# fircarpediem/LSS2_Multimodal_nu

Measured on AMD Instinct MI355X. Metric: BEV frames/sec (6-cam 352x128 -> 200x200x64), full hot path: CamEncode lift + splat + BevEncode, higher is better.
Workload: dtype bf16; 1 GPU; BASELINE configs[1]: model_BEV_TXT LSS hot path, batch=4/GPU, 6 cams 352x128, D=41, 200x200x64 BEV -> BevEncode -> 200x200x4, trunk (EfficientNet) not included: features are the input; batch_per_gpu=4, global_batch=4, parallelism=dp1 (sample-sharded, no collective), precision=bf16

## Files before the change

include/lss_hip.h:

```cpp
#ifndef LSS_HIP_H_
#define LSS_HIP_H_

#include <stddef.h>
#include <stdint.h>

#ifdef __cplusplus
extern "C" {
#endif

#define LSS_ABI_VERSION 1

#define LSS_E_NULL (-1)
#define LSS_E_SHAPE (-2)
#define LSS_E_LAYOUT (-3)
#define LSS_E_ALIGN (-4)
#define LSS_E_WORKSPACE (-5)
#define LSS_E_RCCL_BASE (-100)

#define LSS_BEV_NCHW_F32 0
#define LSS_BEV_NHWC_F32 1
#define LSS_BEV_NHWC_BF16 2

#define LSS_DT_F32 0
#define LSS_DT_BF16 1
// ... 72 lines not shown
                        int n_points, int C, void* workspace, size_t workspace_bytes, float* d_value,
                        float* d_offsets_logits, void* stream);
size_t lss_deform_attn_bwd_workspace_bytes(int B, int H, int W);

int lss_layernorm_fwd(const void* x, int x_dt, const float* gamma, const float* beta,
                      long long rows, int C, float eps, void* y, int y_dt, void* stream);

size_t lss_conv2d_packed_weight_bytes(int Cout, int Cin, int KH, int KW, int dt);
int lss_conv2d_pack_weights(const float* w_oihw, int Cout, int Cin, int KH, int KW,
                            int dt, void* w_packed, void* stream);
int lss_conv2d_fwd(const void* x, const void* x2, const void* w_packed,
                   const float* scale, const float* shift, const void* residual,
                   void* y, float* stats, int B, int H, int W, int Cx, int C2, int up,
                   int Cout, int KH, int KW, int stride, int pad, int relu, int dt,
                   void* stream);

int lss_conv2d_ring_ok(int B, int H, int W, int Cx, int C2, int up, int Cout, int head_n);
size_t lss_conv2d_ring_packed_weight_bytes(int Cout, int Cin);
int lss_conv2d_pack_weights_ring(const float* w_oihw, int Cout, int Cin, void* w_packed, void* stream);
int lss_conv2d_pack_weights_ring_dgrad(const float* w_oihw, int Cout, int Cin, void* w_packed, void* stream);
int lss_conv2d_ring_timeouts(void);

int lss_conv2d_ks_ok(int B, int H, int W, int Cin, int Cout);
size_t lss_conv2d_ks_packed_weight_bytes(int Cout, int Cin);
int lss_conv2d_pack_weights_ks(const float* w_oihw, int Cout, int Cin, void* w_packed, void* stream);
int lss_conv2d_pack_weights_ks_dgrad(const float* w_oihw, int Cout, int Cin, void* w_packed, void* stream);

int lss_conv2d_ks_s2_dual_ok(int B, int H, int W, int Cin, int Cout);
size_t lss_conv2d_ks_s2_dual_packed_weight_bytes(int Cout, int Cin);
int lss_conv2d_pack_weights_ks_s2_dual(const float* w1_oihw, const float* wd_oi, int Cout, int Cin, void* w_packed,
                                       void* stream);
int lss_conv2d_ks_s2_dual_fwd(const void* x, const void* w_packed, const float* scale, const float* shift, void* y,
                              void* y2, int B, int H, int W, int Cin, int Cout, int relu, void* stream);

int lss_conv2d_pack_weights_dgrad(const float* w_oihw, int Cout, int Cin, int KH, int KW, int dt,
                                  void* w_packed, void* stream);
size_t lss_conv2d_wgrad_workspace_bytes(int B, int H, int W, int Cin, int Cout);
int lss_conv2d_wgrad(const void* x, const void* dy, int B, int H, int W, int Cin, int Cout,
                     void* workspace, size_t workspace_bytes, float* dw_oihw, void* stream);
int lss_conv2d_wgrad_timeouts(void);
int lss_conv2d_s2_dgrad_taps(int K, int pad);
int lss_conv2d_pack_weights_s2_dgrad(const float* w_oihw, int Cout, int Cin, int K, int pad, void* w_packed, void* stream);
size_t lss_conv2d_wgrad4x4_workspace_bytes(int B, int H, int W, int Cin, int Cout);
int lss_conv2d_wgrad4x4(const void* xs, const void* dy, int B, int H, int W, int Cin, int Cout,
                        void* workspace, size_t workspace_bytes, float* dw16, void* stream);

int lss_upsample_cat_nhwc(const void* x, const void* x2, int B, int H, int W, int Cx, int C2, int up,
                          void* out, void* stream);
int lss_upsample_bwd_nhwc(const void* g, int B, int H, int W, int Cx, int Ct, int c_off, int up,
                          void* dx, void* stream);

size_t lss_bn_train_workspace_bytes(long long M, int C);
int lss_bn_train_fwd(const void* z, const void* residual, long long M, int C, const float* gamma,
                     const float* beta, float* running_mean, float* running_var, float momentum,
                     float eps, int relu, void* workspace, void* y, float* save_mean,
                     float* save_invstd, void* stream);
int lss_bn_train_bwd(const void* dy, const void* y, const void* z, long long M, int C,
                     const float* gamma, const float* save_mean, const float* save_invstd, int relu,
                     void* workspace, void* dz, void* dres, float* dgamma, float* dbeta, void* stream);

int lss_bn_partial_sums(const void* z, const void* dy, const void* y, const float* mean, const float* invstd,
                        long long M, int C, int relu, int mode, void* workspace, float* sums, void* stream);
int lss_bn_train_fwd_from_sums(const void* z, const void* residual, long long M, int C, const float* sums,
                               long long M_total, const float* gamma, const float* beta, float* running_mean,
                               float* running_var, float momentum, float eps, int relu, void* workspace,
                               void* y, float* save_mean, float* save_invstd, void* stream);
// ... 138 lines not shown
```

lss2_multimodal_nu_amd/_native.py:

```python
import ctypes
import os

import torch

_HERE = os.path.dirname(os.path.abspath(__file__))
LIB_PATH = os.environ.get("LSS_HIP_LIB") or os.path.join(_HERE, "csrc", "liblss_hip.so")

BEV_NCHW_F32, BEV_NHWC_F32, BEV_NHWC_BF16 = 0, 1, 2
DT_F32, DT_BF16 = 0, 1
ACT_NONE, ACT_RELU, ACT_GELU, OUT_F32, OUT_HEAD_MAJOR32, W_RING, W_KS = 0, 1, 2, 16, 32, 64, 128
VALUE_NHWC, VALUE_HEAD_MAJOR = 0, 1

_vp, _i, _sz = ctypes.c_void_p, ctypes.c_int, ctypes.c_size_t

SIGNATURES = {
    "lss_abi_version": (_i, []),
    "lss_error_string": (ctypes.c_char_p, [_i]),
    "lss_points_to_voxels": (_i, [_vp] * 7 + [_i] * 8 + [_vp, _vp, _vp, _vp]),
    "lss_geom_to_voxels": (_i, [_vp, _vp, _vp] + [_i] * 5 + [_vp, _vp, _vp]),
    "lss_bucket_points": (_i, [_vp, _vp, _i, _i, _i, _i, _vp, _vp, _vp, _vp, _vp]),
    "lss_depthnet_softmax_fwd": (_i, [_vp, _vp, _vp, _i, _i, _i, _i, _i, _vp, _vp, _i, _vp]),
    "lss_camencode_v2_fwd": (_i, [_vp, _i, _vp, _vp, _i, _vp, _vp, _vp] + [_i] * 7 + [_vp, _vp, _vp]),
    "lss_depth_fuse_softmax_fwd": (_i, [_vp] * 5 + [_i] * 6 + [_vp, _vp]),
    "lss_add_pos_fwd": (_i, [_vp, _vp, _i, _i, _i, _i, _vp, _vp]),
    "lss_deform_attn_fwd": (_i, [_vp, _i] + [_vp] * 4 + [_i] * 7 + [_vp, _vp]),
    "lss_deform_attn_pts_fwd": (_i, [_vp] * 3 + [ctypes.c_longlong] + [_i] * 6 + [_vp, _vp]),
    "lss_deform_attn_bwd": (_i, [_vp] * 3 + [ctypes.c_longlong, _vp] + [_i] * 6 + [_vp, _sz, _vp, _vp, _vp]),
    "lss_deform_attn_bwd_workspace_bytes": (_sz, [_i] * 3),
    "lss_layernorm_fwd": (_i, [_vp, _i, _vp, _vp, ctypes.c_longlong, _i, ctypes.c_float, _vp, _i, _vp]),
    "lss_depthnet_voxels_fwd": (_i, [_vp] * 10 + [_i] * 10 + [_vp] * 5),
    "lss_linear_res_ln_fwd": (_i, [_vp] * 4 + [ctypes.c_longlong, _i, _vp, _vp, _vp, ctypes.c_float, _vp, _vp]),
    "lss_ffn_fused_fwd": (_i, [_vp] * 5 + [ctypes.c_longlong, _i, _i, _vp, _vp, _vp, ctypes.c_float, _vp, _vp]),
    "lss_depthnet_voxels_hostcal_fwd": (_i, [_vp] * 7 + [_i] * 10 + [_vp] * 5),
    "lss_lift_splat_forward_hostcal": (_i, [_vp] * 7 + [_i] * 10 + [_vp] * 8 + [_i, _vp]),
    "lss_lift_splat_fwd": (_i, [_vp] * 3 + [_i] * 9 + [_vp, _i, _vp]),
    "lss_lift_splat_bwd": (_i, [_vp, _i, _vp, _vp, _vp] + [_i] * 9 + [_vp, _vp]),
    "lss_segmented_sum": (_i, [_vp, _vp, _i, _i, _vp, _vp]),
    "lss_conv2d_packed_weight_bytes": (_sz, [_i] * 5),
    "lss_conv2d_pack_weights": (_i, [_vp, _i, _i, _i, _i, _i, _vp, _vp]),
    "lss_conv2d_fwd": (_i, [_vp] * 8 + [_i] * 13 + [_vp]),
    "lss_conv2d_ring_ok": (_i, [_i] * 8),
    "lss_conv2d_ring_packed_weight_bytes": (_sz, [_i, _i]),
    "lss_conv2d_pack_weights_ring": (_i, [_vp, _i, _i, _vp, _vp]),
    "lss_conv2d_pack_weights_ring_dgrad": (_i, [_vp, _i, _i, _vp, _vp]),
    "lss_conv2d_ks_ok": (_i, [_i] * 5),
    "lss_conv2d_ks_packed_weight_bytes": (_sz, [_i, _i]),
    "lss_conv2d_pack_weights_ks": (_i, [_vp, _i, _i, _vp, _vp]),
    "lss_conv2d_pack_weights_ks_dgrad": (_i, [_vp, _i, _i, _vp, _vp]),
    "lss_conv2d_ks_s2_dual_ok": (_i, [_i] * 5),
    "lss_conv2d_ks_s2_dual_packed_weight_bytes": (_sz, [_i, _i]),
    "lss_conv2d_pack_weights_ks_s2_dual": (_i, [_vp, _vp, _i, _i, _vp, _vp]),
    "lss_conv2d_ks_s2_dual_fwd": (_i, [_vp] * 6 + [_i] * 6 + [_vp]),
    "lss_gather_pack": (_i, [_vp, _i, _vp]),
    "lss_conv_bn_act_train_pack": (_i, [_vp] + [_i] * 8 + [_vp, _vp]),
    "lss_clip_adam_partials": (ctypes.c_longlong, [_vp, _i]),
    "lss_clip_adam_step": (_i, [_vp, _i, _vp, _vp, ctypes.c_longlong] + [ctypes.c_float] * 6 + [_vp]),
    "lss_conv2d_wgrad_timeouts": (_i, []),
    "lss_conv2d_ring_timeouts": (_i, []),
    "lss_conv2d_pack_weights_dgrad": (_i, [_vp, _i, _i, _i, _i, _i, _vp, _vp]),
    "lss_conv2d_wgrad_workspace_bytes": (_sz, [_i] * 5),
    "lss_conv2d_wgrad": (_i, [_vp, _vp, _i, _i, _i, _i, _i, _vp, _sz, _vp, _vp]),
    "lss_conv2d_wgrad4x4_workspace_bytes": (_sz, [_i] * 5),
    "lss_conv2d_s2_dgrad_taps": (_i, [_i, _i]),
    "lss_conv2d_pack_weights_s2_dgrad": (_i, [_vp, _i, _i, _i, _i, _vp, _vp]),
    "lss_conv2d_wgrad4x4": (_i, [_vp, _vp, _i, _i, _i, _i, _i, _vp, _sz, _vp, _vp]),
    "lss_upsample_cat_nhwc": (_i, [_vp, _vp, _i, _i, _i, _i, _i, _i, _vp, _vp]),
    "lss_upsample_bwd_nhwc": (_i, [_vp, _i, _i, _i, _i, _i, _i, _i, _vp, _vp]),
    "lss_bn_train_workspace_bytes": (_sz, [ctypes.c_longlong, _i]),
    "lss_bn_train_fwd": (_i, [_vp, _vp, ctypes.c_longlong, _i, _vp, _vp, _vp, _vp, ctypes.c_float, ctypes.c_float, _i,
                              _vp, _vp, _vp, _vp, _vp]),
    "lss_bn_train_bwd": (_i, [_vp, _vp, _vp, ctypes.c_longlong, _i, _vp, _vp, _vp, _i, _vp, _vp, _vp, _vp, _vp, _vp]),
    "lss_bn_partial_sums": (_i, [_vp] * 5 + [ctypes.c_longlong, _i, _i, _i, _vp, _vp, _vp]),
    "lss_bn_train_fwd_from_sums": (_i, [_vp, _vp, ctypes.c_longlong, _i, _vp, ctypes.c_longlong, _vp, _vp, _vp, _vp,
                                        ctypes.c_float, ctypes.c_float, _i, _vp, _vp, _vp, _vp, _vp]),
    "lss_bn_train_bwd_from_sums": (_i, [_vp, _vp, _vp, ctypes.c_longlong, _i, _vp, ctypes.c_longlong, _vp, _vp, _vp, _i,
                                        _vp, _vp, _vp, _vp, _vp, _vp]),
    "lss_conv_bn_act_train_fwd": (_i, [_vp] * 14 + [_i] * 7 + [ctypes.c_float, ctypes.c_float, _i, _vp]),
    "lss_conv_bn_act_train_bwd": (_i, [_vp] * 11 + [_sz] + [_vp] * 9 + [_i] * 8 + [_vp]),
    "lss_weighted_ce_fwd": (_i, [_vp, _vp, _vp, _i, _i, ctypes.c_longlong, _vp, _vp, _vp, _vp]),
    "lss_weighted_ce_bwd": (_i, [_vp, _vp, _vp, _i, _i, ctypes.c_longlong, _vp, _vp, _vp, _vp]),
    "lss_conv2d_s2d_packed_weight_bytes": (_sz, [_i] * 4),
    "lss_conv2d_pack_weights_s2d": (_i, [_vp, _i, _i, _i, _i, _vp, _vp]),
    "lss_conv2d_s2_fwd": (_i, [_vp] * 7 + [_i] * 8 + [_vp]),
    "lss_conv2d_head_fwd": (_i, [_vp] * 8 + [_i] * 9 + [_vp]),
    "lss_conv2d_s2_dual_fwd": (_i, [_vp] * 6 + [_i] * 9 + [_vp]),
# ... 101 lines not shown
```

lss2_multimodal_nu_amd/csrc/conv_ks.hip:

```cpp
#include <stdlib.h>

#include "lss_common.h"

namespace {

constexpr int KS_ROWS = 7;
constexpr int KS_POSB = 64;
constexpr int KS_LDS_MAX = 160 * 1024;

__device__ __attribute__((aligned(128))) unsigned char lss_ks_zero_page[128];

__device__ __forceinline__ void ks_glds16(const void* gsrc, void* lds_wave_base) {
  __builtin_amdgcn_global_load_lds((const __attribute__((address_space(1))) void*)gsrc,
                                   (__attribute__((address_space(3))) void*)lds_wave_base, 16, 0, 0);
}

struct KsArgs {
  const unsigned short* x;
  const unsigned char* w;
  const float* scale;
  const float* shift;
  const unsigned short* residual;
  unsigned short* y;
  int B, H, W, Cin, Cout, relu, wt;
// ... 517 lines not shown
  const int patch = (Cin / 32) * p.nposp * KS_POSB;
  if (patch > 112 * 1024) return p;
  const int red = 2 * p.nkw * (p.PB / 16) * KS2_CT * 1024;
  p.lds = patch > red ? patch : red;
  if (p.lds > KS_LDS_MAX) return p;
  const long long grid = (long long)B * p.npb * p.ncb;
  if (grid < 64 || grid > 512) return p;
  if ((long long)B * H * W * Cin >= (1LL << 30) || (long long)B * HWo * Cout >= (1LL << 30)) return p;
  p.grid = (int)grid;
  p.ok = 1;
  return p;
}

template <int NKW>
int ks_s2_launch(const KsS2Plan& p, const KsS2Args& a, hipStream_t st) {
  static bool attr_set[64] = {};
  int dev = -1;
  if (hipGetDevice(&dev) != hipSuccess || dev < 0 || dev >= 64) dev = -1;
  if (dev < 0 || !attr_set[dev]) {
    hipError_t e = hipFuncSetAttribute(reinterpret_cast<const void*>(conv_ks_s2_dual_kernel<NKW>),
                                       hipFuncAttributeMaxDynamicSharedMemorySize, KS_LDS_MAX);
    if (e != hipSuccess) return (int)e;
    if (dev >= 0) attr_set[dev] = true;
  }
  hipLaunchKernelGGL((conv_ks_s2_dual_kernel<NKW>), dim3(p.grid), dim3(256), p.lds, st, a);
  return lss_launch_status();
}

unsigned long long* ks_stamps_from_env() {
  const char* e = getenv("LSS_KS_STAMPS");
  return e ? reinterpret_cast<unsigned long long*>(strtoull(e, nullptr, 16)) : nullptr;
}

}

extern "C" int lss_conv2d_ks_ok(int B, int H, int W, int Cin, int Cout) {
  if (const char* e = getenv("LSS_CONV_KS"))
    if (atoi(e) == 0) return 0;
  return ks_plan(B, H, W, Cin, Cout).ok;
}

extern "C" size_t lss_conv2d_ks_packed_weight_bytes(int Cout, int Cin) {
  if (Cout <= 0 || Cout % 32 != 0 || (Cin != 64 && Cin != 128 && Cin != 256)) return 0;
  return (size_t)Cout * Cin * 9 * 2;
}

extern "C" int lss_conv2d_pack_weights_ks(const float* w_oihw, int Cout, int Cin, void* w_packed, void* stream) {
  LSS_CHECK_PTR(w_oihw); LSS_CHECK_PTR(w_packed);
  if (lss_conv2d_ks_packed_weight_bytes(Cout, Cin) == 0) return LSS_E_SHAPE;
  const size_t n = (size_t)Cout * Cin * 9;
  const int grid = (int)((n + 255) / 256 > 4096 ? 4096 : (n + 255) / 256);
  hipLaunchKernelGGL(pack_weights_ks_kernel, dim3(grid), dim3(256), 0, lss_stream(stream), w_oihw, Cout, Cin,
                     reinterpret_cast<unsigned short*>(w_packed), 0);
  return lss_launch_status();
}

extern "C" int lss_conv2d_pack_weights_ks_dgrad(const float* w_oihw, int Cout, int Cin, void* w_packed, void* stream) {
  LSS_CHECK_PTR(w_oihw); LSS_CHECK_PTR(w_packed);
  if (lss_conv2d_ks_packed_weight_bytes(Cin, Cout) == 0) return LSS_E_SHAPE;
  const size_t n = (size_t)Cout * Cin * 9;
  const int grid = (int)((n + 255) / 256 > 4096 ? 4096 : (n + 255) / 256);
  hipLaunchKernelGGL(pack_weights_ks_kernel, dim3(grid), dim3(256), 0, lss_stream(stream), w_oihw, Cin, Cout,
                     reinterpret_cast<unsigned short*>(w_packed), 1);
  return lss_launch_status();
}

// ... 33 lines not shown
extern "C" int lss_conv2d_pack_weights_ks_s2_dual(const float* w1_oihw, const float* wd_oi, int Cout, int Cin,
                                                  void* w_packed, void* stream) {
  LSS_CHECK_PTR(w1_oihw); LSS_CHECK_PTR(wd_oi); LSS_CHECK_PTR(w_packed);
  if (lss_conv2d_ks_s2_dual_packed_weight_bytes(Cout, Cin) == 0) return LSS_E_SHAPE;
  const size_t n = (size_t)Cout * Cin * 10;
  const int grid = (int)((n + 255) / 256 > 4096 ? 4096 : (n + 255) / 256);
  hipLaunchKernelGGL(pack_weights_ks_s2_dual_kernel, dim3(grid), dim3(256), 0, lss_stream(stream), w1_oihw, wd_oi, Cout,
                     Cin, reinterpret_cast<unsigned short*>(w_packed));
  return lss_launch_status();
}

extern "C" int lss_conv2d_ks_s2_dual_fwd(const void* x, const void* w_packed, const float* scale, const float* shift,
                                         void* y, void* y2, int B, int H, int W, int Cin, int Cout, int relu,
                                         void* stream) {
  LSS_CHECK_PTR(x); LSS_CHECK_PTR(w_packed); LSS_CHECK_PTR(y); LSS_CHECK_PTR(y2);
  const KsS2Plan p = ks_s2_plan(B, H, W, Cin, Cout);
  if (!p.ok) return LSS_E_SHAPE;
  if (relu != 0 && relu != 1) return LSS_E_LAYOUT;
  if (((reinterpret_cast<uintptr_t>(x) | reinterpret_cast<uintptr_t>(y) | reinterpret_cast<uintptr_t>(y2) |
        reinterpret_cast<uintptr_t>(w_packed) | reinterpret_cast<uintptr_t>(scale) | reinterpret_cast<uintptr_t>(shift)) & 15) != 0)
    return LSS_E_ALIGN;
  KsS2Args a;
  a.x = reinterpret_cast<const unsigned short*>(x);
  a.w = reinterpret_cast<const unsigned char*>(w_packed);
  a.scale = scale; a.shift = shift;
  a.y = reinterpret_cast<unsigned short*>(y);
  a.y2 = reinterpret_cast<unsigned short*>(y2);
  a.B = B; a.H = H; a.W = W; a.Cin = Cin; a.Cout = Cout; a.relu = relu;
  a.Ho = p.Ho; a.Wo = p.Wo; a.pitch = p.pitch;
  a.PB = p.PB; a.npb = p.npb; a.nposp = p.nposp; a.ncb = p.ncb;
  a.stamps = ks_stamps_from_env();
  return p.nkw == 4 ? ks_s2_launch<4>(p, a, lss_stream(stream)) : ks_s2_launch<2>(p, a, lss_stream(stream));
}
```

lss2_multimodal_nu_amd/csrc/conv_mfma.hip:

```cpp
#include <stdlib.h>

#include "lss_common.h"

int lss_linear_bf16_launch(const void* x, const void* w, const float* scale, const float* shift,
                           const void* residual, void* y, long long M, int N, int K, int act,
                           int out_f32, int group_hw, hipStream_t st);

int lss_conv_ring_launch(const void* x, const void* x2, const void* w_ring, const float* scale, const float* shift,
                         void* y, const float* head_w, const float* head_b, float* head_out, int head_n, int B, int H,
                         int W, int Cx, int C2, int up, int Cout, int relu, int wt, hipStream_t st);

int lss_conv_ks_launch(const void* x, const void* w_ks, const float* scale, const float* shift, const void* residual,
                       void* y, int B, int H, int W, int Cin, int Cout, int relu, int wt, hipStream_t st);

namespace {

struct ConvArgs {
  const void* x;
  const void* x2;
  const void* w;
  const float* scale;
  const float* shift;
  const void* residual;
  void* y;
// ... 1183 lines not shown
  if (fused && kc32) {
    a.src_lds = conv_src_lds_ok(a);
    hipLaunchKernelGGL((conv_lds_kernel<2, 128, 1, 3, 3, 1, 32, 1, true>), g, dim3(256), 0, st, a, tilesX, tilesY);
  }
  else if (fused)
    hipLaunchKernelGGL((conv_lds_kernel<2, 128, 1, 3, 3, 1, 64, 1, true>), g, dim3(256), 0, st, a, tilesX, tilesY);
  else if (Cout == 64)
    hipLaunchKernelGGL((conv_lds_kernel<2, 64, 0, 3, 3, 1, 64, 1, true>), g, dim3(256), 0, st, a, tilesX, tilesY);
  else
    hipLaunchKernelGGL((conv_lds_kernel<2, 128, 0, 3, 3, 1, 64, 1, true>), g, dim3(256), 0, st, a, tilesX, tilesY);
  return lss_launch_status();
}

extern "C" int lss_conv2d_sequence(const lss_conv_launch_t* L, int n, void* stream) {
  LSS_CHECK_PTR(L);
  if (n < 0) return LSS_E_SHAPE;
  for (int i = 0; i < n; ++i) {
    const lss_conv_launch_t& c = L[i];
    int rc;
    if (c.kind == 0)
      rc = lss_conv2d_fwd(c.x, c.x2, c.w, c.scale, c.shift, c.residual, c.y, c.stats, c.B, c.H, c.W, c.Cx,
                          c.C2, c.up, c.Cout, c.KH, c.KW, c.stride, c.pad, c.relu, c.dt, stream);
    else if (c.kind == 1)
      rc = lss_conv2d_s2_fwd(c.x, c.w, c.scale, c.shift, c.residual, c.y, c.stats, c.B, c.H, c.W, c.Cx,
                             c.Cout, c.KH, c.pad, c.relu, stream);
    else if (c.kind == 2)
      rc = lss_conv2d_head_fwd(c.x, c.x2, c.w, c.scale, c.shift, c.head_w, c.head_b, c.head_out, c.B, c.H,
                               c.W, c.Cx, c.C2, c.up, c.Cout, c.head_n, c.relu, stream);
    else if (c.kind == 3)
      rc = lss_conv2d_s2_dual_fwd(c.x, c.w, c.scale, c.shift, c.y, c.y2, c.B, c.H, c.W, c.Cx, c.Cout, c.split, c.KH,
                                  c.pad, c.relu, stream);
    else if (c.kind == 4)
      rc = lss_conv2d_ks_s2_dual_fwd(c.x, c.w, c.scale, c.shift, c.y, c.y2, c.B, c.H, c.W, c.Cx, c.Cout, c.relu, stream);
    else
      rc = LSS_E_LAYOUT;
    if (rc != 0) return rc;
  }
  return 0;
}
```

lss2_multimodal_nu_amd/modules.py:

```python
import os

import torch
from torch import nn
from torch.nn import functional as F

from . import ops

_PRECISIONS = {"bf16": ops.DT_BF16, "fp32": ops.DT_F32}


def default_precision():
    p = os.environ.get("LSS_PRECISION", "bf16")
    if p not in _PRECISIONS:
        raise ValueError("LSS_PRECISION must be one of %s" % sorted(_PRECISIONS))
    return p


_warned_eval_autograd = set()


def _needs_autograd(module, *inputs):
    if not torch.is_grad_enabled():
        return False
    in_grad = any(t is not None and torch.is_tensor(t) and t.requires_grad for t in inputs)
# ... 403 lines not shown
def _train_up_conv(conv, up, x1, x2):
    c2 = 0 if x2 is None else x2.shape[1]
    if (x1.is_cuda and conv.kernel_size == (3, 3) and conv.stride == (1, 1) and conv.padding == (1, 1)
            and conv.bias is None and x1.shape[1] % 64 == 0 and c2 % 64 == 0 and conv.out_channels % 8 == 0
            and x1.shape[2] > 1 and x1.shape[3] > 1 and _native_training()):
        return _UpConv3x3Fn.apply(x1, x2, conv.weight, int(up.scale_factor))
    x1 = up(x1)
    return _train_conv(conv, x1 if x2 is None else torch.cat([x2, x1], dim=1))


def _train_conv(conv, x):
    if (x.is_cuda and conv.kernel_size == (3, 3) and conv.stride == (1, 1) and conv.padding == (1, 1)
            and conv.dilation == (1, 1) and conv.groups == 1 and conv.bias is None
            and conv.in_channels % 64 == 0 and conv.out_channels % 8 == 0 and _native_training()):
        return _Conv3x3Fn.apply(x, conv.weight)
    k, p = conv.kernel_size[0], conv.padding[0]
    if (x.is_cuda and conv.stride == (2, 2) and conv.kernel_size in ((1, 1), (3, 3), (7, 7)) and conv.padding == (k // 2, k // 2)
            and conv.dilation == (1, 1) and conv.groups == 1 and conv.bias is None and conv.in_channels % 64 == 0
            and conv.out_channels % 64 == 0 and x.shape[2] % 2 == 0 and x.shape[3] % 2 == 0 and _native_training()):
        return _ConvS2Fn.apply(x, conv.weight, p)
    return conv(x)


class _FoldedConv:

    def __init__(self, conv, bn=None, pack=True, pad_in=None):
        self.conv, self.bn = conv, bn
        self.pack = pack
        self.pad_in = pad_in
        self.key = None
        self.w = self.scale = self.shift = None
        self.w_ring, self.ring_key = None, None
        self.w_ks, self.ks_key = None, None

    def ks(self, dt):
        if self.ks_key != self.key:
            with torch.no_grad():
                self.w_ks = ops.pack_conv_weight_ks(self.conv.weight.detach().float().contiguous())
            self.ks_key = self.key
        return self.w_ks

    def ks_case(self, x, dt, x2=None, up=1):
        c = self.conv
        if (dt != ops.DT_BF16 or x2 is not None or up != 1 or c.kernel_size != (3, 3) or c.stride != (1, 1)
                or c.padding != (1, 1) or not self.pack or self.pad_in is not None):
            return False
        B, H, W, Cx = x.shape
        return ops.conv_ks_ok(B, H, W, Cx, c.out_channels)

    def ring(self, dt):
        if self.ring_key != self.key:
            with torch.no_grad():
                w32 = self.conv.weight.detach().float().contiguous()
                if self.pad_in is not None:
                    at, n = self.pad_in
                    w32 = torch.cat([w32[:, :at], w32.new_zeros(w32.shape[0], n, *w32.shape[2:]), w32[:, at:]],
                                    1).contiguous()
                self.w_ring = ops.pack_conv_weight_ring(w32)
            self.ring_key = self.key
        return self.w_ring

    def ring_case(self, x, dt, residual=None, x2=None, up=1, head_n=0):
        c = self.conv
        if (dt != ops.DT_BF16 or residual is not None or c.kernel_size != (3, 3) or c.stride != (1, 1)
                or c.padding != (1, 1) or not self.pack):
            return False
# ... 16 lines not shown
                and c.padding[0] == c.kernel_size[0] // 2 and c.in_channels % 64 == 0)

    def get(self, dt):
        key = self._key(dt)
        if key != self.key:
            with torch.no_grad():
                w32 = self.conv.weight.detach().float().contiguous()
                if self.pad_in is not None:
                    at, n = self.pad_in
                    w32 = torch.cat([w32[:, :at], w32.new_zeros(w32.shape[0], n, *w32.shape[2:]), w32[:, at:]],
                                    1).contiguous()
                if not self.pack:
                    self.w = None
                elif self._s2d(dt) and self.conv.kernel_size[0] > 1:
                    self.w = ops.pack_conv_weight_s2d(w32, self.conv.padding[0])
                else:
                    self.w = ops.pack_conv_weight(w32, dt)
                if self.bn is not None:
                    inv = torch.rsqrt(self.bn.running_var.float() + self.bn.eps)
                    self.scale = (self.bn.weight.float() * inv).contiguous()
                    mean = self.bn.running_mean.float()
                    if self.conv.bias is not None:
                        mean = mean - self.conv.bias.detach().float()
                    self.shift = (self.bn.bias.float() - mean * self.scale).contiguous()
                else:
                    self.scale = None
                    self.shift = self.conv.bias.detach().float().contiguous() if self.conv.bias is not None else None
            self.key = key
        return self.w, self.scale, self.shift

    def run(self, x, dt, relu, residual=None, x2=None, up=1):
        w, scale, shift = self.get(dt)
        c = self.conv
        if self._s2d(dt) and x2 is None and up == 1:
            return ops.conv2d_s2_nhwc(x, w, c.kernel_size[0], c.padding[0], scale, shift, residual, relu)
        if relu in (False, True) and self.ks_case(x, dt, x2, up):
            w = self.ks(dt)
        elif relu in (False, True) and self.ring_case(x, dt, residual, x2, up):
            w = self.ring(dt)
        return ops.conv2d_nhwc(x, w, c.kernel_size, c.stride[0], c.padding[0], scale, shift, residual, relu,
                               x2=x2, up=up, dt=dt)


def _to_nhwc(x, dt):
    if x.dtype == torch.bfloat16 and dt == ops.DT_BF16 and x.is_contiguous(memory_format=torch.channels_last):
        return x.permute(0, 2, 3, 1)
    x = x.float()
    if dt == ops.DT_F32 and x.is_contiguous(memory_format=torch.channels_last) and not x.is_contiguous():
        return x.permute(0, 2, 3, 1)
    return ops.nchw_to_nhwc(x.contiguous(), dt)


class Up(nn.Module):

    def __init__(self, in_channels, out_channels, scale_factor=2, precision=None):
        super().__init__()
        self.up = nn.Upsample(scale_factor=scale_factor, mode="bilinear", align_corners=True)
        self.conv = nn.Sequential(
            nn.Conv2d(in_channels, out_channels, kernel_size=3, padding=1, bias=False),
            nn.BatchNorm2d(out_channels),
            nn.ReLU(inplace=True),
            nn.Conv2d(out_channels, out_channels, kernel_size=3, padding=1, bias=False),
            nn.BatchNorm2d(out_channels),
            nn.ReLU(inplace=True))
        self.scale_factor = int(scale_factor)
        self.precision = precision
# ... 314 lines not shown
```

lss2_multimodal_nu_amd/ops.py:

```python
import ctypes
import os
import threading

import torch

from . import _native as N
from ._native import (ACT_GELU, ACT_NONE, ACT_RELU, BEV_NCHW_F32, BEV_NHWC_BF16, BEV_NHWC_F32, DT_BF16,
                      DT_F32, OUT_F32, OUT_HEAD_MAJOR32, VALUE_HEAD_MAJOR, VALUE_NHWC, W_KS, W_RING)


def _f32c(t, name, shape=None):
    if t.dtype != torch.float32 or not t.is_contiguous() or not t.is_cuda:
        raise ValueError("%s must be a contiguous fp32 GPU tensor (got %s %s contiguous=%s)"
                         % (name, t.dtype, t.device, t.is_contiguous()))
    if shape is not None and tuple(t.shape) != tuple(shape):
        raise ValueError("%s has shape %s, expected %s" % (name, tuple(t.shape), tuple(shape)))
    return t


class KernelTimer:

    def __init__(self, fine=False, last_conv=False):
        self.spans = {}
        self.fine = fine
# ... 1206 lines not shown
    _f32c(wd_oihw, "downsample weight", (Cout, Cin, 1, 1))
    nbytes = N.lib().lss_conv2d_ks_s2_dual_packed_weight_bytes(Cout, Cin)
    if (KH, KW) != (3, 3) or nbytes == 0:
        raise ValueError("KS stride-2 weights: 3x3 + 1x1, Cout %% 64 == 0, Cin in (64, 128) (got %s)"
                         % (tuple(w1_oihw.shape),))
    out = torch.empty(nbytes // 2, dtype=torch.bfloat16, device=w1_oihw.device)
    N.check(N.lib().lss_conv2d_pack_weights_ks_s2_dual(N.ptr(w1_oihw), N.ptr(wd_oihw), Cout, Cin, N.ptr(out),
                                                       N.stream()), "lss_conv2d_pack_weights_ks_s2_dual")
    return KsWeight(out, Cout, Cin)


def conv2d_ks_s2_dual_nhwc(x, w_ks, scale=None, shift=None, relu=True, tag="conv2d_fwd"):
    B, H, W, Cx = x.shape
    if x.dtype != torch.bfloat16 or not x.is_contiguous() or not isinstance(w_ks, KsWeight) or w_ks.Cin != Cx \
            or w_ks.data.numel() != w_ks.Cout * Cx * 10:
        raise ValueError("conv2d_ks_s2_dual_nhwc operands must be contiguous bf16 with stride-2 KS-packed weights")
    Cout = w_ks.Cout
    for name, t in (("scale", scale), ("shift", shift)):
        if t is not None:
            _f32c(t, name, (2 * Cout,))
    Ho, Wo = (H - 1) // 2 + 1, (W - 1) // 2 + 1
    y = torch.empty(B, Ho, Wo, Cout, dtype=torch.bfloat16, device=x.device)
    y2 = torch.empty(B, Ho, Wo, Cout, dtype=torch.bfloat16, device=x.device)
    if _recorder is not None:
        _recorder.add(4, (x, w_ks.data, scale, shift, y, y2), x=x, w=w_ks.data, scale=scale, shift=shift, y=y, y2=y2,
                      B=B, H=H, W=W, Cx=Cx, Cout=Cout, KH=3, KW=3, stride=2, pad=1, relu=1 if relu else 0, dt=DT_BF16)
    with _timed(tag):
        N.check(N.lib().lss_conv2d_ks_s2_dual_fwd(N.ptr(x), N.ptr(w_ks.data), N.ptr(scale), N.ptr(shift), N.ptr(y),
                                                  N.ptr(y2), B, H, W, Cx, Cout, 1 if relu else 0, N.stream()),
                "lss_conv2d_ks_s2_dual_fwd")
    return y, y2


def conv3x3_head_nchw(x, w_packed, scale, shift, head_w, head_b, x2=None, up=1, relu=True, tag="conv2d_fwd"):
    B, H, W, Cx = x.shape
    ring = isinstance(w_packed, RingWeight)
    if ring:
        taps, Cout, Cin, w_packed = 9, w_packed.Cout, w_packed.Cin, w_packed.data
    else:
        taps, Cout, Cin = w_packed.shape
    C2 = x2.shape[3] if x2 is not None else 0
    if x.dtype != torch.bfloat16 or not x.is_contiguous() or taps != 9 or Cin != Cx + C2 or Cout not in (64, 128) \
            or (Cout == 64 and (up != 1 or C2 != 0)):
        raise ValueError("conv3x3_head_nchw: bf16 NHWC input, 3x3 weights with Cout == 128 (or 64 without "
                         "upsample / concat) required")
    n = head_w.shape[0]
    _f32c(head_w, "head_w", (n, Cout))
    _f32c(head_b, "head_b", (n,))
    _f32c(scale, "scale", (Cout,))
    _f32c(shift, "shift", (Cout,))
    out = torch.empty(B, n, H * up, W * up, dtype=torch.float32, device=x.device)
    if _recorder is not None:
        _recorder.add(2, (x, x2, w_packed, scale, shift, head_w, head_b, out), x=x, x2=x2, w=w_packed, scale=scale,
                      shift=shift, head_w=head_w, head_b=head_b, head_out=out, B=B, H=H, W=W, Cx=Cx, C2=C2, up=up,
                      Cout=Cout, KH=3, KW=3, stride=1, pad=1, relu=(1 if relu else 0) | (W_RING if ring else 0),
                      dt=DT_BF16, head_n=n)
    with _timed(tag):
        N.check(N.lib().lss_conv2d_head_fwd(N.ptr(x), N.ptr(x2), N.ptr(w_packed), N.ptr(scale), N.ptr(shift),
                                            N.ptr(head_w), N.ptr(head_b), N.ptr(out), B, H, W, Cx, C2, up, Cout, n,
                                            (1 if relu else 0) | (W_RING if ring else 0), N.stream()),
                "lss_conv2d_head_fwd")
    return out


def nchw_to_nhwc(x, dt):
    _f32c(x, "x")
# ... 14 lines not shown
```

Measured before the change: 11570 frames/s.

## Add dedicated MFMA kernel for 7x7 stride-2 BevEncode stem conv

Adds a specialized bf16 MFMA kernel for the 7x7 stride-2 Cin=64 stem convolution in BevEncode. It stages an input patch into LDS via direct global-to-LDS loads, with even and odd columns split so stride-2 taps read contiguously. Weights are held in registers and prefetched ahead across 98 K-steps, and BN scale/shift plus ReLU are fused into the epilogue. The aim is to replace the generic or space-to-depth stride-2 path for this layer, at the cost of heavy register use (launch bounds allow one block per CU) and a grid restricted to 32-256 blocks.

```diff
diff --git a/include/lss_hip.h b/include/lss_hip.h
--- a/include/lss_hip.h
+++ b/include/lss_hip.h
@@ -128,6 +128,12 @@
                                        void* stream);
 int lss_conv2d_ks_s2_dual_fwd(const void* x, const void* w_packed, const float* scale, const float* shift, void* y,
                               void* y2, int B, int H, int W, int Cin, int Cout, int relu, void* stream);
+
+int lss_conv2d_ks_stem_ok(int B, int H, int W, int Cin, int Cout);
+size_t lss_conv2d_ks_stem_packed_weight_bytes(int Cout, int Cin);
+int lss_conv2d_pack_weights_ks_stem(const float* w_oihw, int Cout, int Cin, void* w_packed, void* stream);
+int lss_conv2d_ks_stem_fwd(const void* x, const void* w_packed, const float* scale, const float* shift, void* y,
+                           int B, int H, int W, int Cin, int Cout, int relu, void* stream);
 
 int lss_conv2d_pack_weights_dgrad(const float* w_oihw, int Cout, int Cin, int KH, int KW, int dt,
                                   void* w_packed, void* stream);
diff --git a/lss2_multimodal_nu_amd/_native.py b/lss2_multimodal_nu_amd/_native.py
--- a/lss2_multimodal_nu_amd/_native.py
+++ b/lss2_multimodal_nu_amd/_native.py
@@ -51,6 +51,10 @@
     "lss_conv2d_ks_s2_dual_packed_weight_bytes": (_sz, [_i, _i]),
     "lss_conv2d_pack_weights_ks_s2_dual": (_i, [_vp, _vp, _i, _i, _vp, _vp]),
     "lss_conv2d_ks_s2_dual_fwd": (_i, [_vp] * 6 + [_i] * 6 + [_vp]),
+    "lss_conv2d_ks_stem_ok": (_i, [_i] * 5),
+    "lss_conv2d_ks_stem_packed_weight_bytes": (_sz, [_i, _i]),
+    "lss_conv2d_pack_weights_ks_stem": (_i, [_vp, _i, _i, _vp, _vp]),
+    "lss_conv2d_ks_stem_fwd": (_i, [_vp] * 5 + [_i] * 6 + [_vp]),
     "lss_gather_pack": (_i, [_vp, _i, _vp]),
     "lss_conv_bn_act_train_pack": (_i, [_vp] + [_i] * 8 + [_vp, _vp]),
     "lss_clip_adam_partials": (ctypes.c_longlong, [_vp, _i]),
diff --git a/lss2_multimodal_nu_amd/csrc/conv_ks.hip b/lss2_multimodal_nu_amd/csrc/conv_ks.hip
--- a/lss2_multimodal_nu_amd/csrc/conv_ks.hip
+++ b/lss2_multimodal_nu_amd/csrc/conv_ks.hip
@@ -573,6 +573,191 @@
   return e ? reinterpret_cast<unsigned long long*>(strtoull(e, nullptr, 16)) : nullptr;
 }
 
+constexpr int ST_TH = 12, ST_TW = 16;
+constexpr int ST_PR = 2 * ST_TH + 5, ST_PW = 2 * ST_TW + 5;
+constexpr int ST_NE = ST_TW + 3;
+constexpr int ST_NPOSP = (ST_PR * ST_PW + 31) / 32 * 32;
+constexpr int ST_LDS = 2 * ST_NPOSP * KS_POSB;
+constexpr int ST_KS = 98;
+constexpr int ST_WPRE = 8;
+constexpr int ST_PXT = ST_TH / 2;
+
+struct KsStemArgs {
+  const unsigned short* x;
+  const unsigned char* w;
+  const float* scale;
+  const float* shift;
+  unsigned short* y;
+  int B, H, W, Cout, relu;
+  int Ho, Wo, nty, ntx, ncb;
+  unsigned long long* stamps;
+};
+
+__global__ __launch_bounds__(256, 1) void conv_ks_stem_kernel(const KsStemArgs a) {
+  constexpr int PXT = ST_PXT, Cin = 64;
+  extern __shared__ __attribute__((aligned(1024))) unsigned char smem[];
+  const int tid = threadIdx.x, lane = tid & 63;
+  const int wave = __builtin_amdgcn_readfirstlane(tid >> 6);
+  const int g = wave & 1, ph = wave >> 1;
+  const int n = lane & 15, kq = lane >> 4;
+  auto stamp = [&](int k) {
+    if (a.stamps != nullptr && tid == 0) a.stamps[(size_t)blockIdx.x * 8 + k] = __builtin_amdgcn_s_memrealtime();
+  };
+  stamp(0);
+  unsigned long long clk_main = 0;
+
+  int t;
+  {
+    const int nwg = gridDim.x, bid = blockIdx.x;
+    const int xcd = bid & 7, q8 = nwg >> 3, r8 = nwg & 7;
+    t = (xcd < r8 ? xcd * (q8 + 1) : r8 * (q8 + 1) + (xcd - r8) * q8) + (bid >> 3);
+  }
+  const int cb = t % a.ncb;
+  const int tg = t / a.ncb;
+  const int npi = a.nty * a.ntx;
+  const int b = tg / npi, ti = tg - b * npi;
+  const int ty = ti / a.ntx, tx = ti - ty * a.ntx;
+  const int oy0 = ty * ST_TH, ox0 = tx * ST_TW;
+  const int iy0 = 2 * oy0 - 3, ix0 = 2 * ox0 - 3;
+
+  {
+    constexpr int ppc = ST_NPOSP >> 4;
+    constexpr int q64 = 64 / ST_PW, r64 = 64 - q64 * ST_PW;
+    const int h = wave & 1;
+    const int pos0 = 32 * (wave >> 1) + (lane >> 1);
+    int pr = pos0 / ST_PW, pc = pos0 - pr * ST_PW;
+    const unsigned char* zsrc = lss_ks_zero_page + (lane & 7) * 16;
+    const unsigned short* xb = a.x + (size_t)b * a.H * a.W * Cin + (2 * h + (lane & 1)) * 8;
+    for (int i = wave; i < ppc; i += 4) {
+      const int iy = iy0 + pr, ix = ix0 + (pc < ST_NE ? 2 * pc : 2 * (pc - ST_NE) + 1);
+      const bool in = pr < ST_PR && iy >= 0 && iy < a.H && ix >= 0 && ix < a.W;
+      const unsigned short* src = xb + (in ? (iy * a.W + ix) * Cin : 0);
+#pragma unroll
+      for (int c = 0; c < 2; ++c)
+        ks_glds16(in ? (const void*)(src + c * 32) : (const void*)zsrc,
+                  smem + ((size_t)(c * 2 + h) * ST_NPOSP + 32 * (i >> 1)) * 32);
+      pr += q64; pc += r64;
+      if (pc >= ST_PW) { pc -= ST_PW; ++pr; }
+    }
+  }
+
+  bf16x8 wf[ST_KS][2];
+  const unsigned char* wp = a.w + ((size_t)cb * ST_KS * 4 + 2 * g) * 1024 + lane * 16;
+  auto load_w = [&](int s) {
+#pragma unroll
+    for (int ct = 0; ct < 2; ++ct) wf[s][ct] = *reinterpret_cast<const bf16x8*>(wp + (s * 4 + ct) * 1024);
+  };
+#pragma unroll
+  for (int s = 0; s < ST_WPRE; ++s) load_w(s);
+
+  const int ab0 = (2 * (ph * PXT) * ST_PW + n) * 32 + (kq >> 1) * ST_NPOSP * 32 + (kq & 1) * 16;
+  stamp(1);
+  f32x4 acc[PXT][2];
+#pragma unroll
+  for (int j = 0; j < PXT; ++j) {
+    acc[j][0] = (f32x4){0.f, 0.f, 0.f, 0.f};
+    acc[j][1] = (f32x4){0.f, 0.f, 0.f, 0.f};
+  }
+  const int ch = cb * 64 + g * 32 + kq * 8;
+  float sc[8], sh[8];
+  {
+    f32x4 s0 = {1.f, 1.f, 1.f, 1.f}, s1 = s0, h0 = {0.f, 0.f, 0.f, 0.f}, h1 = h0;
+    if (a.scale) { s0 = *reinterpret_cast<const f32x4*>(a.scale + ch); s1 = *reinterpret_cast<const f32x4*>(a.scale + ch + 4); }
+    if (a.shift) { h0 = *reinterpret_cast<const f32x4*>(a.shift + ch); h1 = *reinterpret_cast<const f32x4*>(a.shift + ch + 4); }
+#pragma unroll
+    for (int i = 0; i < 4; ++i) { sc[i] = s0[i]; sc[4 + i] = s1[i]; sh[i] = h0[i]; sh[4 + i] = h1[i]; }
+  }
+  asm volatile("s_waitcnt vmcnt(0)" ::: "memory");
+  __syncthreads();
+  stamp(2);
+
+  bf16x8 fb[2][PXT];
+  auto load_frags = [&](int buf, int s) {
+    const int tap = s >> 1, ky = tap / 7, kx = tap % 7;
+    const int toff = (ky * ST_PW + ((kx & 1) ? ST_NE + (kx >> 1) : (kx >> 1))) * 32;
+    const unsigned char* cbase = smem + (size_t)(s & 1) * 2 * ST_NPOSP * 32 + ab0 + toff;
+#pragma unroll
+    for (int j = 0; j < PXT; ++j) fb[buf][j] = *reinterpret_cast<const bf16x8*>(cbase + j * (2 * ST_PW * 32));
+  };
+  if (a.stamps != nullptr) clk_main = __builtin_amdgcn_s_memtime();
+  load_frags(0, 0);
+#pragma unroll
+  for (int s = 0; s < ST_KS; ++s) {
+    if (s + ST_WPRE < ST_KS) load_w(s + ST_WPRE);
+    if (s + 1 < ST_KS) load_frags((s + 1) & 1, s + 1);
+    __builtin_amdgcn_sched_barrier(0);
+#pragma unroll
+    for (int j = 0; j < PXT; ++j) {
+      acc[j][0] = __builtin_amdgcn_mfma_f32_16x16x32_bf16(wf[s][0], fb[s & 1][j], acc[j][0], 0, 0, 0);
+      acc[j][1] = __builtin_amdgcn_mfma_f32_16x16x32_bf16(wf[s][1], fb[s & 1][j], acc[j][1], 0, 0, 0);
+    }
+    __builtin_amdgcn_sched_barrier(0);
+  }
+  if (a.stamps != nullptr) asm volatile("s_nop 0" ::"v"(acc[0][0]), "v"(acc[PXT - 1][1]));
+  stamp(3);
+  if (a.stamps != nullptr && tid == 0) a.stamps[(size_t)blockIdx.x * 8 + 7] = __builtin_amdgcn_s_memtime() - clk_main;
+  stamp(4);
+
+  const int ox = ox0 + n;
+#pragma unroll
+  for (int j = 0; j < PXT; ++j) {
+    const int oy = oy0 + ph * PXT + j;
+    float v[8];
+#pragma unroll
+    for (int i = 0; i < 4; ++i) { v[i] = acc[j][0][i]; v[4 + i] = acc[j][1][i]; }
+#pragma unroll
+    for (int i = 0; i < 8; ++i) {
+      v[i] = v[i] * sc[i] + sh[i];
+      if (a.relu) v[i] = fmaxf(v[i], 0.f);
+    }
+    if (oy < a.Ho && ox < a.Wo) {
+      typedef __attribute__((ext_vector_type(4))) unsigned int u32x4;
+      const u32x4 ov = {lss_pack_bf2(v[0], v[1]), lss_pack_bf2(v[2], v[3]), lss_pack_bf2(v[4], v[5]), lss_pack_bf2(v[6], v[7])};
+      *reinterpret_cast<u32x4*>(a.y + (((size_t)b * a.Ho + oy) * a.Wo + ox) * a.Cout + ch) = ov;
+    }
+  }
+  if (a.stamps != nullptr) {
+    stamp(5);
+    asm volatile("s_waitcnt vmcnt(0)" ::: "memory");
+    stamp(6);
+  }
+}
+
+__global__ void pack_weights_ks_stem_kernel(const float* __restrict__ w, int Cout, unsigned short* __restrict__ out) {
+  const size_t ntot = (size_t)Cout * 64 * 49;
+  for (size_t e = (size_t)blockIdx.x * 256 + threadIdx.x; e < ntot; e += (size_t)gridDim.x * 256) {
+    const int j = e & 7;
+    size_t r = e >> 3;
+    const int l = r & 63; r >>= 6;
+    const int ct = r & 3; r >>= 2;
+    const int S = r % ST_KS;
+    const int cb = r / ST_KS;
+    const int m = l & 15, kq = l >> 4;
+    const int co = cb * 64 + 32 * (ct >> 1) + 8 * (m >> 2) + 4 * (ct & 1) + (m & 3);
+    const int ci = (S & 1) * 32 + kq * 8 + j;
+    out[e] = lss_f2bf(w[((size_t)co * 64 + ci) * 49 + (S >> 1)]);
+  }
+}
+
+struct KsStemPlan {
+  int ok, Ho, Wo, nty, ntx, ncb, grid;
+};
+
+KsStemPlan ks_stem_plan(int B, int H, int W, int Cin, int Cout) {
+  KsStemPlan p = {};
+  if (B <= 0 || H <= 0 || W <= 0 || Cin != 64 || Cout <= 0 || Cout % 64 != 0) return p;
+  p.Ho = (H - 1) / 2 + 1; p.Wo = (W - 1) / 2 + 1;
+  if (p.Ho < ST_TH || p.Wo < ST_TW) return p;
+  p.nty = (p.Ho + ST_TH - 1) / ST_TH; p.ntx = (p.Wo + ST_TW - 1) / ST_TW;
+  p.ncb = Cout / 64;
+  const long long grid = (long long)B * p.nty * p.ntx * p.ncb;
+  if (grid < 32 || grid > 256) return p;
+  if ((long long)B * H * W * Cin >= (1LL << 30) || (long long)B * p.Ho * p.Wo * Cout >= (1LL << 30)) return p;
+  p.grid = (int)grid;
+  p.ok = 1;
+  return p;
+}
+
 }
 
 extern "C" int lss_conv2d_ks_ok(int B, int H, int W, int Cin, int Cout) {
@@ -672,3 +857,54 @@
   a.stamps = ks_stamps_from_env();
   return p.nkw == 4 ? ks_s2_launch<4>(p, a, lss_stream(stream)) : ks_s2_launch<2>(p, a, lss_stream(stream));
 }
+
+extern "C" int lss_conv2d_ks_stem_ok(int B, int H, int W, int Cin, int Cout) {
+  if (const char* e = getenv("LSS_CONV_KS"))
+    if (atoi(e) == 0) return 0;
+  return ks_stem_plan(B, H, W, Cin, Cout).ok;
+}
+
+extern "C" size_t lss_conv2d_ks_stem_packed_weight_bytes(int Cout, int Cin) {
+  if (Cout <= 0 || Cout % 64 != 0 || Cin != 64) return 0;
+  return (size_t)Cout * Cin * 49 * 2;
+}
+
+extern "C" int lss_conv2d_pack_weights_ks_stem(const float* w_oihw, int Cout, int Cin, void* w_packed, void* stream) {
+  LSS_CHECK_PTR(w_oihw); LSS_CHECK_PTR(w_packed);
+  if (lss_conv2d_ks_stem_packed_weight_bytes(Cout, Cin) == 0) return LSS_E_SHAPE;
+  const size_t n = (size_t)Cout * Cin * 49;
+  const int grid = (int)((n + 255) / 256 > 4096 ? 4096 : (n + 255) / 256);
+  hipLaunchKernelGGL(pack_weights_ks_stem_kernel, dim3(grid), dim3(256), 0, lss_stream(stream), w_oihw, Cout,
+                     reinterpret_cast<unsigned short*>(w_packed));
+  return lss_launch_status();
+}
+
+extern "C" int lss_conv2d_ks_stem_fwd(const void* x, const void* w_packed, const float* scale, const float* shift,
+                                      void* y, int B, int H, int W, int Cin, int Cout, int relu, void* stream) {
+  LSS_CHECK_PTR(x); LSS_CHECK_PTR(w_packed); LSS_CHECK_PTR(y);
+  const KsStemPlan p = ks_stem_plan(B, H, W, Cin, Cout);
+  if (!p.ok) return LSS_E_SHAPE;
+  if (relu != 0 && relu != 1) return LSS_E_LAYOUT;
+  if (((reinterpret_cast<uintptr_t>(x) | reinterpret_cast<uintptr_t>(y) | reinterpret_cast<uintptr_t>(w_packed) |
+        reinterpret_cast<uintptr_t>(scale) | reinterpret_cast<uintptr_t>(shift)) & 15) != 0)
+    return LSS_E_ALIGN;
+  KsStemArgs a;
+  a.x = reinterpret_cast<const unsigned short*>(x);
+  a.w = reinterpret_cast<const unsigned char*>(w_packed);
+  a.scale = scale; a.shift = shift;
+  a.y = reinterpret_cast<unsigned short*>(y);
+  a.B = B; a.H = H; a.W = W; a.Cout = Cout; a.relu = relu;
+  a.Ho = p.Ho; a.Wo = p.Wo; a.nty = p.nty; a.ntx = p.ntx; a.ncb = p.ncb;
+  a.stamps = ks_stamps_from_env();
+  static bool attr_set[64] = {};
+  int dev = -1;
+  if (hipGetDevice(&dev) != hipSuccess || dev < 0 || dev >= 64) dev = -1;
+  if (dev < 0 || !attr_set[dev]) {
+    hipError_t e = hipFuncSetAttribute(reinterpret_cast<const void*>(conv_ks_stem_kernel),
+                                       hipFuncAttributeMaxDynamicSharedMemorySize, KS_LDS_MAX);
+    if (e != hipSuccess) return (int)e;
+    if (dev >= 0) attr_set[dev] = true;
+  }
+  hipLaunchKernelGGL(conv_ks_stem_kernel, dim3(p.grid), dim3(256), ST_LDS, lss_stream(stream), a);
+  return lss_launch_status();
+}
diff --git a/lss2_multimodal_nu_amd/csrc/conv_mfma.hip b/lss2_multimodal_nu_amd/csrc/conv_mfma.hip
--- a/lss2_multimodal_nu_amd/csrc/conv_mfma.hip
+++ b/lss2_multimodal_nu_amd/csrc/conv_mfma.hip
@@ -1239,6 +1239,8 @@
                                   c.pad, c.relu, stream);
     else if (c.kind == 4)
       rc = lss_conv2d_ks_s2_dual_fwd(c.x, c.w, c.scale, c.shift, c.y, c.y2, c.B, c.H, c.W, c.Cx, c.Cout, c.relu, stream);
+    else if (c.kind == 5)
+      rc = lss_conv2d_ks_stem_fwd(c.x, c.w, c.scale, c.shift, c.y, c.B, c.H, c.W, c.Cx, c.Cout, c.relu, stream);
     else
       rc = LSS_E_LAYOUT;
     if (rc != 0) return rc;
diff --git a/lss2_multimodal_nu_amd/modules.py b/lss2_multimodal_nu_amd/modules.py
--- a/lss2_multimodal_nu_amd/modules.py
+++ b/lss2_multimodal_nu_amd/modules.py
@@ -459,6 +459,23 @@
         self.w = self.scale = self.shift = None
         self.w_ring, self.ring_key = None, None
         self.w_ks, self.ks_key = None, None
+        self.w_stem, self.stem_key = None, None
+
+    def stem(self, dt):
+        if self.stem_key != self.key:
+            with torch.no_grad():
+                self.w_stem = ops.pack_conv_weight_ks_stem(self.conv.weight.detach().float().contiguous())
+            self.stem_key = self.key
+        return self.w_stem
+
+    def stem_case(self, x, dt, residual=None, x2=None, up=1):
+        c = self.conv
+        if (dt != ops.DT_BF16 or residual is not None or x2 is not None or up != 1 or c.kernel_size != (7, 7)
+                or c.stride != (2, 2) or c.padding != (3, 3) or not self.pack or self.pad_in is not None
+                or os.environ.get("LSS_NO_STEM_KS") is not None):
+            return False
+        B, H, W, Cx = x.shape
+        return ops.conv_ks_stem_ok(B, H, W, Cx, c.out_channels)
 
     def ks(self, dt):
         if self.ks_key != self.key:
@@ -541,6 +558,8 @@
     def run(self, x, dt, relu, residual=None, x2=None, up=1):
         w, scale, shift = self.get(dt)
         c = self.conv
+        if relu in (False, True) and self.stem_case(x, dt, residual, x2, up):
+            return ops.conv2d_ks_stem_nhwc(x, self.stem(dt), scale, shift, relu=relu)
         if self._s2d(dt) and x2 is None and up == 1:
             return ops.conv2d_s2_nhwc(x, w, c.kernel_size[0], c.padding[0], scale, shift, residual, relu)
         if relu in (False, True) and self.ks_case(x, dt, x2, up):
diff --git a/lss2_multimodal_nu_amd/ops.py b/lss2_multimodal_nu_amd/ops.py
--- a/lss2_multimodal_nu_amd/ops.py
+++ b/lss2_multimodal_nu_amd/ops.py
@@ -1262,6 +1262,43 @@
     return y, y2
 
 
+def conv_ks_stem_ok(B, H, W, Cin, Cout):
+    return bool(N.lib().lss_conv2d_ks_stem_ok(B, H, W, Cin, Cout))
+
+
+def pack_conv_weight_ks_stem(w_oihw):
+    Cout, Cin, KH, KW = w_oihw.shape
+    _f32c(w_oihw, "conv weight")
+    nbytes = N.lib().lss_conv2d_ks_stem_packed_weight_bytes(Cout, Cin)
+    if (KH, KW) != (7, 7) or nbytes == 0:
+        raise ValueError("KS stem weights: 7x7, Cout %% 64 == 0, Cin 64 (got %s)" % (tuple(w_oihw.shape),))
+    out = torch.empty(nbytes // 2, dtype=torch.bfloat16, device=w_oihw.device)
+    N.check(N.lib().lss_conv2d_pack_weights_ks_stem(N.ptr(w_oihw), Cout, Cin, N.ptr(out), N.stream()),
+            "lss_conv2d_pack_weights_ks_stem")
+    return KsWeight(out, Cout, Cin)
+
+
+def conv2d_ks_stem_nhwc(x, w_ks, scale=None, shift=None, relu=True, tag="conv2d_fwd"):
+    B, H, W, Cx = x.shape
+    if x.dtype != torch.bfloat16 or not x.is_contiguous() or not isinstance(w_ks, KsWeight) or w_ks.Cin != Cx \
+            or w_ks.data.numel() != w_ks.Cout * Cx * 49:
+        raise ValueError("conv2d_ks_stem_nhwc operands must be contiguous bf16 with stem KS-packed weights")
+    Cout = w_ks.Cout
+    for name, t in (("scale", scale), ("shift", shift)):
+        if t is not None:
+            _f32c(t, name, (Cout,))
+    Ho, Wo = (H - 1) // 2 + 1, (W - 1) // 2 + 1
+    y = torch.empty(B, Ho, Wo, Cout, dtype=torch.bfloat16, device=x.device)
+    if _recorder is not None:
+        _recorder.add(5, (x, w_ks.data, scale, shift, y), x=x, w=w_ks.data, scale=scale, shift=shift, y=y,
+                      B=B, H=H, W=W, Cx=Cx, Cout=Cout, KH=7, KW=7, stride=2, pad=3, relu=1 if relu else 0, dt=DT_BF16)
+    with _timed(tag):
+        N.check(N.lib().lss_conv2d_ks_stem_fwd(N.ptr(x), N.ptr(w_ks.data), N.ptr(scale), N.ptr(shift), N.ptr(y),
+                                               B, H, W, Cx, Cout, 1 if relu else 0, N.stream()),
+                "lss_conv2d_ks_stem_fwd")
+    return y
+
+
 def conv3x3_head_nchw(x, w_packed, scale, shift, head_w, head_b, x2=None, up=1, relu=True, tag="conv2d_fwd"):
     B, H, W, Cx = x.shape
     ring = isinstance(w_packed, RingWeight)
```

New measurement: 11990 frames/s, median of 6. +3.6%, better.
